# icdm-adteam/MoCoPCI

Hardware: AMD Instinct MI355X
Metric: interpolated frames/sec (higher is better)
Workload: dtype f32 (fused MLP layers: fp32 products as 6 bf16-MFMA partials of an exact 3-way split, fp32 accumulate; index paths exact f32)

## Files before the change

mocopci_amd/csrc/pointconv.hip:

```cpp
#include "common.h"
#include "mfma_split.h"

namespace {

constexpr int K = 32, WN = 8;

template <int THREADS, int PPB>
__global__ __launch_bounds__(THREADS) void pointconv_agg_kernel(long long total, int n, int s, int d, const float *__restrict__ s_xyz,
                                                                const float *__restrict__ new_xyz, const float *__restrict__ s_points,
                                                                const int *__restrict__ idx, const float *__restrict__ w0,
                                                                const float *__restrict__ b0, const float *__restrict__ w1,
                                                                const float *__restrict__ b1, const float *__restrict__ w2,
                                                                const float *__restrict__ b2, float *__restrict__ out) {
    __shared__ __attribute__((aligned(16))) float wl[PPB][K][WN];
    __shared__ float gx[PPB][K][3];
    __shared__ int il[PPB][K];
    const int tid = threadIdx.x;
    const int cin = d + 3;
    const bool f32 = mcp_fits32(total);
    const bool off32 = (long long)n * d < (1LL << 31);
    const int d4 = d >> 2;
    const McpUnits units = mcp_units_by_xcd(total, PPB);
    for (long long p0 = units.first; p0 < units.limit; p0 += units.stride) {
        __syncthreads();
        for (int pair = tid; pair < PPB * K; pair += THREADS) {
            const int pl = pair >> 5, k = pair & 31;
            const long long p = p0 + pl;
            if (p < total) {
                const long long bb = mcp_div(p, s, f32);
                const int id = idx[p * K + k];
                const float *q = s_xyz + ((long long)bb * n + id) * 3;
                const float x0 = q[0] - new_xyz[p * 3 + 0], x1 = q[1] - new_xyz[p * 3 + 1], x2 = q[2] - new_xyz[p * 3 + 2];
                float h0[WN], h1[WN], h2[WN];
#pragma unroll
                for (int j = 0; j < WN; ++j)
                    h0[j] = fmaxf(__builtin_fmaf(w0[j * 3 + 2], x2, __builtin_fmaf(w0[j * 3 + 1], x1, __builtin_fmaf(w0[j * 3], x0, b0[j]))), 0.f);
#pragma unroll
                for (int j = 0; j < WN; ++j) {
                    float a = b1[j];
#pragma unroll
                    for (int i = 0; i < WN; ++i) a = __builtin_fmaf(w1[j * WN + i], h0[i], a);
                    h1[j] = fmaxf(a, 0.f);
                }
#pragma unroll
                for (int j = 0; j < WN; ++j) {
                    float a = b2[j];
#pragma unroll
                    for (int i = 0; i < WN; ++i) a = __builtin_fmaf(w2[j * WN + i], h1[i], a);
                    h2[j] = fmaxf(a, 0.f);
                }
#pragma unroll
                for (int j = 0; j < WN; ++j) wl[pl][k][j] = h2[j];
                gx[pl][k][0] = x0; gx[pl][k][1] = x1; gx[pl][k][2] = x2;
                il[pl][k] = id;
            }
        }
        __syncthreads();
        for (int it = tid; it < PPB * d4; it += THREADS) {
            const int pl = it / d4, c = (it - pl * d4) * 4;
            const long long p = p0 + pl;
            if (p >= total) break;
            const long long bb = mcp_div(p, s, f32);
            float acc[4][WN];
#pragma unroll
            for (int u = 0; u < 4; ++u)
#pragma unroll
                for (int j = 0; j < WN; ++j) acc[u][j] = 0.f;
            const float *fb = s_points + (long long)bb * n * d + c;
#pragma unroll 8
            for (int k = 0; k < K; ++k) {
                const float4 f = *reinterpret_cast<const float4 *>(off32 ? fb + (unsigned)il[pl][k] * (unsigned)d : fb + (long long)il[pl][k] * d);
                const float4 wa = *reinterpret_cast<const float4 *>(&wl[pl][k][0]);
                const float4 wb = *reinterpret_cast<const float4 *>(&wl[pl][k][4]);
                const float fv[4] = {f.x, f.y, f.z, f.w};
#pragma unroll
                for (int u = 0; u < 4; ++u) {
                    acc[u][0] = __builtin_fmaf(fv[u], wa.x, acc[u][0]); acc[u][1] = __builtin_fmaf(fv[u], wa.y, acc[u][1]);
                    acc[u][2] = __builtin_fmaf(fv[u], wa.z, acc[u][2]); acc[u][3] = __builtin_fmaf(fv[u], wa.w, acc[u][3]);
                    acc[u][4] = __builtin_fmaf(fv[u], wb.x, acc[u][4]); acc[u][5] = __builtin_fmaf(fv[u], wb.y, acc[u][5]);
                    acc[u][6] = __builtin_fmaf(fv[u], wb.z, acc[u][6]); acc[u][7] = __builtin_fmaf(fv[u], wb.w, acc[u][7]);
                }
            }
            float4 *o = reinterpret_cast<float4 *>(out + (p * cin + 3 + c) * WN);
#pragma unroll
            for (int u = 0; u < 4; ++u) {
                o[2 * u] = make_float4(acc[u][0], acc[u][1], acc[u][2], acc[u][3]);
                o[2 * u + 1] = make_float4(acc[u][4], acc[u][5], acc[u][6], acc[u][7]);
            }
        }
        if (tid < PPB * 3) {
            const int pl = tid / 3, c = tid - pl * 3;
            const long long p = p0 + pl;
            if (p < total) {
                float acc[WN];
#pragma unroll
                for (int j = 0; j < WN; ++j) acc[j] = 0.f;
#pragma unroll 8
                for (int k = 0; k < K; ++k) {
                    const float f = gx[pl][k][c];
                    const float4 wa = *reinterpret_cast<const float4 *>(&wl[pl][k][0]);
                    const float4 wb = *reinterpret_cast<const float4 *>(&wl[pl][k][4]);
                    acc[0] = __builtin_fmaf(f, wa.x, acc[0]); acc[1] = __builtin_fmaf(f, wa.y, acc[1]);
                    acc[2] = __builtin_fmaf(f, wa.z, acc[2]); acc[3] = __builtin_fmaf(f, wa.w, acc[3]);
                    acc[4] = __builtin_fmaf(f, wb.x, acc[4]); acc[5] = __builtin_fmaf(f, wb.y, acc[5]);
                    acc[6] = __builtin_fmaf(f, wb.z, acc[6]); acc[7] = __builtin_fmaf(f, wb.w, acc[7]);
                }
                float4 *o = reinterpret_cast<float4 *>(out + (p * cin + c) * WN);
                o[0] = make_float4(acc[0], acc[1], acc[2], acc[3]);
                o[1] = make_float4(acc[4], acc[5], acc[6], acc[7]);
            }
        }
    }
}

constexpr int LPPB = 8;
template <int THREADS>
__global__ __launch_bounds__(THREADS) void pointconv_agg_lowlevel_kernel(long long total, int n, int s, int d, const float *__restrict__ s_xyz,
                                                                const float *__restrict__ new_xyz, const float *__restrict__ s_points,
                                                                const int *__restrict__ idx, const float *__restrict__ w0,
                                                                const float *__restrict__ b0, const float *__restrict__ w1,
                                                                const float *__restrict__ b1, const float *__restrict__ w2,
                                                                const float *__restrict__ b2, float *__restrict__ out) {
    __shared__ __attribute__((aligned(16))) float wl[LPPB][K][WN];
    __shared__ float gx[LPPB][K][3];
    __shared__ int il[LPPB][K];
    const int tid = threadIdx.x;
    const int cin = d + 3;
    const bool f32 = mcp_fits32(total);
    const bool off32 = (long long)n * d < (1LL << 31);
    const McpUnits units = mcp_units_by_xcd(total, LPPB);
    for (long long p0 = units.first; p0 < units.limit; p0 += units.stride) {
        __syncthreads();
        {
            const int pl = tid >> 5, k = tid & 31;
            const long long p = p0 + pl;
            if (tid < LPPB * K && p < total) {
                const long long bb = mcp_div(p, s, f32);
                const int id = idx[p * K + k];
                const float *q = s_xyz + ((long long)bb * n + id) * 3;
                const float x0 = q[0] - new_xyz[p * 3 + 0], x1 = q[1] - new_xyz[p * 3 + 1], x2 = q[2] - new_xyz[p * 3 + 2];
                float h0[WN], h1[WN], h2[WN];
#pragma unroll
                for (int j = 0; j < WN; ++j)
                    h0[j] = fmaxf(__builtin_fmaf(w0[j * 3 + 2], x2, __builtin_fmaf(w0[j * 3 + 1], x1, __builtin_fmaf(w0[j * 3], x0, b0[j]))), 0.f);
#pragma unroll
                for (int j = 0; j < WN; ++j) {
                    float a = b1[j];
#pragma unroll
                    for (int i = 0; i < WN; ++i) a = __builtin_fmaf(w1[j * WN + i], h0[i], a);
                    h1[j] = fmaxf(a, 0.f);
                }
#pragma unroll
                for (int j = 0; j < WN; ++j) {
                    float a = b2[j];
#pragma unroll
                    for (int i = 0; i < WN; ++i) a = __builtin_fmaf(w2[j * WN + i], h1[i], a);
                    h2[j] = fmaxf(a, 0.f);
                }
#pragma unroll
                for (int j = 0; j < WN; ++j) wl[pl][k][j] = h2[j];
                gx[pl][k][0] = x0; gx[pl][k][1] = x1; gx[pl][k][2] = x2;
                il[pl][k] = id;
            }
        }
        __syncthreads();
        for (int it = tid; it < LPPB * d; it += THREADS) {
            const int pl = it / d, c = it - pl * d;
            const long long p = p0 + pl;
            if (p >= total) break;
            const long long bb = mcp_div(p, s, f32);
            float acc[WN];
#pragma unroll
            for (int j = 0; j < WN; ++j) acc[j] = 0.f;
            const float *fb = s_points + (long long)bb * n * d + c;
#pragma unroll 8
            for (int k = 0; k < K; ++k) {
                const float f = off32 ? fb[(unsigned)il[pl][k] * (unsigned)d] : fb[(long long)il[pl][k] * d];
                const float4 wa = *reinterpret_cast<const float4 *>(&wl[pl][k][0]);
                const float4 wb = *reinterpret_cast<const float4 *>(&wl[pl][k][4]);
                acc[0] = __builtin_fmaf(f, wa.x, acc[0]); acc[1] = __builtin_fmaf(f, wa.y, acc[1]);
                acc[2] = __builtin_fmaf(f, wa.z, acc[2]); acc[3] = __builtin_fmaf(f, wa.w, acc[3]);
                acc[4] = __builtin_fmaf(f, wb.x, acc[4]); acc[5] = __builtin_fmaf(f, wb.y, acc[5]);
                acc[6] = __builtin_fmaf(f, wb.z, acc[6]); acc[7] = __builtin_fmaf(f, wb.w, acc[7]);
            }
            float4 *o = reinterpret_cast<float4 *>(out + (p * cin + 3 + c) * WN);
            o[0] = make_float4(acc[0], acc[1], acc[2], acc[3]);
            o[1] = make_float4(acc[4], acc[5], acc[6], acc[7]);
        }
        if (tid < LPPB * 3) {
            const int pl = tid / 3, c = tid - pl * 3;
            const long long p = p0 + pl;
            if (p < total) {
                float acc[WN];
#pragma unroll
                for (int j = 0; j < WN; ++j) acc[j] = 0.f;
#pragma unroll 8
                for (int k = 0; k < K; ++k) {
                    const float f = gx[pl][k][c];
                    const float4 wa = *reinterpret_cast<const float4 *>(&wl[pl][k][0]);
                    const float4 wb = *reinterpret_cast<const float4 *>(&wl[pl][k][4]);
                    acc[0] = __builtin_fmaf(f, wa.x, acc[0]); acc[1] = __builtin_fmaf(f, wa.y, acc[1]);
                    acc[2] = __builtin_fmaf(f, wa.z, acc[2]); acc[3] = __builtin_fmaf(f, wa.w, acc[3]);
                    acc[4] = __builtin_fmaf(f, wb.x, acc[4]); acc[5] = __builtin_fmaf(f, wb.y, acc[5]);
                    acc[6] = __builtin_fmaf(f, wb.z, acc[6]); acc[7] = __builtin_fmaf(f, wb.w, acc[7]);
                }
                float4 *o = reinterpret_cast<float4 *>(out + (p * cin + c) * WN);
                o[0] = make_float4(acc[0], acc[1], acc[2], acc[3]);
                o[1] = make_float4(acc[4], acc[5], acc[6], acc[7]);
            }
        }
    }
}

constexpr int FPPB = 32;
template <int D, int NT>
struct FusedCfg {
    static constexpr int THREADS = 8 * D;
    static constexpr int KTOT = 8 * D + 24, NCH = (KTOT + 31) / 32, KP = NCH * 32 + 4;
    static constexpr int SCRATCH_BYTES = FPPB * K * (WN + 3 + 1) * 4;
    static constexpr int TILE_BYTES = FPPB * KP * 4;
    static constexpr int XP = 36;
    static constexpr int STAGE_BYTES = NT * 32 * XP * 4;
    static constexpr int LDS_BYTES = (SCRATCH_BYTES > TILE_BYTES + STAGE_BYTES ? SCRATCH_BYTES : TILE_BYTES + STAGE_BYTES);
    static_assert(NT <= THREADS / 64, "one wave per output tile");
    static_assert(2 * LDS_BYTES <= 160 * 1024 || D < 64, "two workgroups per CU");
};

template <int D, int NT>
__global__ __launch_bounds__(8 * D) __attribute__((amdgpu_waves_per_eu(D == 32 ? 3 : 4))) void pointconv_linear_kernel(long long total, int n, int s, const float *__restrict__ s_xyz,
                                                                  const float *__restrict__ new_xyz, const float *__restrict__ s_points,
                                                                  const int *__restrict__ idx, const float *__restrict__ w0,
                                                                  const float *__restrict__ b0, const float *__restrict__ w1,
                                                                  const float *__restrict__ b1, const float *__restrict__ w2,
                                                                  const float *__restrict__ b2, const float *__restrict__ packed, int cout,
                                                                  float slope, float *__restrict__ out) {
    using C = FusedCfg<D, NT>;
    constexpr int THREADS = C::THREADS, NCH = C::NCH, KP = C::KP, KTOT = C::KTOT, D4 = D / 4, XP = C::XP;
    constexpr int CF = NT * 2 * 3 * 64 * 4;
    constexpr int UNR = D == 32 ? 4 : 2;
    extern __shared__ __attribute__((aligned(16))) float flds[];
    float(*wl)[K][WN] = reinterpret_cast<float(*)[K][WN]>(flds);
    float(*gx)[K][3] = reinterpret_cast<float(*)[K][3]>(flds + FPPB * K * WN);
    int(*il)[K] = reinterpret_cast<int(*)[K]>(flds + FPPB * K * (WN + 3));
    float *tile = flds;
    const int tid = threadIdx.x, lane = tid & 63, wave = tid >> 6, h = lane >> 5, col = lane & 31;
    const bool f32 = mcp_fits32(total);
    const bool off32 = (long long)n * D < (1LL << 31);
    const McpUnits units = mcp_units_by_xcd(total, FPPB);
    for (long long p0 = units.first; p0 < units.limit; p0 += units.stride) {
        __syncthreads();
        for (int pair = tid; pair < FPPB * K; pair += THREADS) {
            const int pl = pair >> 5, k = pair & 31;
            const long long p = p0 + pl;
            if (p < total) {
                const long long bb = mcp_div(p, s, f32);
                const int id = idx[p * K + k];
                const float *q = s_xyz + ((long long)bb * n + id) * 3;
                const float x0 = q[0] - new_xyz[p * 3 + 0], x1 = q[1] - new_xyz[p * 3 + 1], x2 = q[2] - new_xyz[p * 3 + 2];
                float h0[WN], h1[WN], h2[WN];
#pragma unroll
                for (int j = 0; j < WN; ++j)
                    h0[j] = fmaxf(__builtin_fmaf(w0[j * 3 + 2], x2, __builtin_fmaf(w0[j * 3 + 1], x1, __builtin_fmaf(w0[j * 3], x0, b0[j]))), 0.f);
#pragma unroll
                for (int j = 0; j < WN; ++j) {
                    float a = b1[j];
#pragma unroll
                    for (int i = 0; i < WN; ++i) a = __builtin_fmaf(w1[j * WN + i], h0[i], a);
                    h1[j] = fmaxf(a, 0.f);
                }
#pragma unroll
                for (int j = 0; j < WN; ++j) {
                    float a = b2[j];
#pragma unroll
                    for (int i = 0; i < WN; ++i) a = __builtin_fmaf(w2[j * WN + i], h1[i], a);
                    h2[j] = fmaxf(a, 0.f);
                }
#pragma unroll
                for (int j = 0; j < WN; ++j) wl[pl][k][j] = h2[j];
                gx[pl][k][0] = x0; gx[pl][k][1] = x1; gx[pl][k][2] = x2;
                il[pl][k] = id;
            }
        }
        __syncthreads();
        const int pl = tid / D4, c4 = tid - pl * D4;
        float acc[4][WN], accx[WN];
#pragma unroll
        for (int u = 0; u < 4; ++u)
#pragma unroll
            for (int j = 0; j < WN; ++j) acc[u][j] = 0.f;
#pragma unroll
        for (int j = 0; j < WN; ++j) accx[j] = 0.f;
        if (p0 + pl < total) {
            const long long bb = mcp_div(p0 + pl, s, f32);
            const float *fb = s_points + (long long)bb * n * D + c4 * 4;
#pragma unroll UNR
            for (int k = 0; k < K; ++k) {
                const float4 f = *reinterpret_cast<const float4 *>(off32 ? fb + (unsigned)il[pl][k] * (unsigned)D : fb + (long long)il[pl][k] * D);
                const float4 wa = *reinterpret_cast<const float4 *>(&wl[pl][k][0]);
                const float4 wb = *reinterpret_cast<const float4 *>(&wl[pl][k][4]);
                const float fv[4] = {f.x, f.y, f.z, f.w};
#pragma unroll
                for (int u = 0; u < 4; ++u) {
                    acc[u][0] = __builtin_fmaf(fv[u], wa.x, acc[u][0]); acc[u][1] = __builtin_fmaf(fv[u], wa.y, acc[u][1]);
                    acc[u][2] = __builtin_fmaf(fv[u], wa.z, acc[u][2]); acc[u][3] = __builtin_fmaf(fv[u], wa.w, acc[u][3]);
                    acc[u][4] = __builtin_fmaf(fv[u], wb.x, acc[u][4]); acc[u][5] = __builtin_fmaf(fv[u], wb.y, acc[u][5]);
                    acc[u][6] = __builtin_fmaf(fv[u], wb.z, acc[u][6]); acc[u][7] = __builtin_fmaf(fv[u], wb.w, acc[u][7]);
                }
            }
        }
        const int xl = tid / 3, xc = tid - xl * 3;
        if (tid < FPPB * 3 && p0 + xl < total) {
#pragma unroll UNR
            for (int k = 0; k < K; ++k) {
                const float f = gx[xl][k][xc];
                const float4 wa = *reinterpret_cast<const float4 *>(&wl[xl][k][0]);
                const float4 wb = *reinterpret_cast<const float4 *>(&wl[xl][k][4]);
                accx[0] = __builtin_fmaf(f, wa.x, accx[0]); accx[1] = __builtin_fmaf(f, wa.y, accx[1]);
                accx[2] = __builtin_fmaf(f, wa.z, accx[2]); accx[3] = __builtin_fmaf(f, wa.w, accx[3]);
                accx[4] = __builtin_fmaf(f, wb.x, accx[4]); accx[5] = __builtin_fmaf(f, wb.y, accx[5]);
                accx[6] = __builtin_fmaf(f, wb.z, accx[6]); accx[7] = __builtin_fmaf(f, wb.w, accx[7]);
            }
        }
        struct Wts { uint4 w[2][3]; };
        auto request = [&](int c, Wts &g) {
            const uint4 *wc = reinterpret_cast<const uint4 *>(packed + (size_t)min(c, NCH - 1) * CF) + (size_t)min(wave, NT - 1) * 2 * 3 * 64 + lane;
#pragma unroll
            for (int s2 = 0; s2 < 2; ++s2)
#pragma unroll
                for (int pc = 0; pc < 3; ++pc) g.w[s2][pc] = wc[(size_t)(s2 * 3 + pc) * 64];
        };
        Wts wa_;
        if (wave < NT) request(0, wa_);
        __syncthreads();
        {
            float *row = tile + pl * KP + 24 + c4 * 32;
#pragma unroll
            for (int u = 0; u < 4; ++u) {
                *reinterpret_cast<float4 *>(row + 8 * u) = make_float4(acc[u][0], acc[u][1], acc[u][2], acc[u][3]);
                *reinterpret_cast<float4 *>(row + 8 * u + 4) = make_float4(acc[u][4], acc[u][5], acc[u][6], acc[u][7]);
            }
            if (tid < FPPB * 3) {
                float *xr = tile + xl * KP + xc * 8;
                *reinterpret_cast<float4 *>(xr) = make_float4(accx[0], accx[1], accx[2], accx[3]);
                *reinterpret_cast<float4 *>(xr + 4) = make_float4(accx[4], accx[5], accx[6], accx[7]);
            } else if (tid < FPPB * 3 + FPPB) {
                float *xr = tile + (tid - FPPB * 3) * KP + KTOT;
#pragma unroll
                for (int i = 0; i < NCH * 32 - KTOT; i += 4) *reinterpret_cast<float4 *>(xr + i) = make_float4(0.f, 0.f, 0.f, 0.f);
            }
        }
        __syncthreads();
        if (wave < NT) {
            mcp_f32x16 o;
            {
                const float *bi = packed + (size_t)NCH * CF;
#pragma unroll
                for (int r = 0; r < 16; ++r) o[r] = bi[(wave * 2 + h) * 16 + r];
            }
#pragma unroll 1
            for (int c = 0; c < NCH; ++c) {
                mcp_f32x16 xa;
#pragma unroll
                for (int g = 0; g < 4; ++g) {
                    const float4 v = *reinterpret_cast<const float4 *>(tile + col * KP + c * 32 + 8 * g + 4 * h);
                    xa[4 * g + 0] = v.x; xa[4 * g + 1] = v.y; xa[4 * g + 2] = v.z; xa[4 * g + 3] = v.w;
                }
                McpSplit3 xs[2];
                xs[0] = mcp_split_kstep(xa, 0);
                xs[1] = mcp_split_kstep(xa, 1);
#pragma unroll
                for (int s2 = 0; s2 < 2; ++s2) {
                    o = mcp_mfma_bf16(wa_.w[s2][2], xs[s2].p1, o);
                    o = mcp_mfma_bf16(wa_.w[s2][0], xs[s2].p3, o);
                    o = mcp_mfma_bf16(wa_.w[s2][1], xs[s2].p2, o);
                    o = mcp_mfma_bf16(wa_.w[s2][1], xs[s2].p1, o);
                    o = mcp_mfma_bf16(wa_.w[s2][0], xs[s2].p2, o);
                    o = mcp_mfma_bf16(wa_.w[s2][0], xs[s2].p1, o);
                }
                request(c + 1, wa_);
            }
            float *st = flds + C::TILE_BYTES / 4 + wave * 32 * XP;
#pragma unroll
            for (int g = 0; g < 4; ++g) {
                float v[4];
#pragma unroll
                for (int u = 0; u < 4; ++u) {
                    const float a = o[4 * g + u];
                    v[u] = a > 0.f ? a : a * slope;
                }
                *reinterpret_cast<float4 *>(st + col * XP + 8 * g + 4 * h) = make_float4(v[0], v[1], v[2], v[3]);
            }
            const int cr = lane >> 3, cq = lane & 7;
#pragma unroll
            for (int j = 0; j < 4; ++j) {
                const long long p = p0 + 8 * j + cr;
                const float4 v4 = *reinterpret_cast<const float4 *>(st + (8 * j + cr) * XP + 4 * cq);
                if (p < total) *reinterpret_cast<float4 *>(out + p * cout + 32 * wave + 4 * cq) = v4;
            }
        }
    }
}

}

MCP_EXPORT int mcp_pointconv_agg(int b, int n, int s, int d, int k, const float *s_xyz, const float *new_xyz, const float *s_points,
                                 const int *idx, const float *w0, const float *b0, const float *w1, const float *b1, const float *w2,
                                 const float *b2, float *out, mcp_stream_t stream) {
    MCP_CHECK_ARGS(b > 0 && n > 0 && s > 0 && d > 0 && s_xyz && new_xyz && s_points && idx && w0 && b0 && w1 && b1 && w2 && b2 && out);
    if (k != K) return MCP_ERR_UNSUPPORTED;
    if (((uintptr_t)out) & 15) return MCP_ERR_BAD_ARG;
    hipStream_t st = (hipStream_t)stream;
    const long long total = (long long)b * s;
    const bool vec4 = !(d & 3) && !(((uintptr_t)s_points) & 15);
    mcp_prof_begin(MCP_KERNEL_POINTCONV, st);
    auto launch = [&](auto kern, int ppb) {
        const unsigned grid = (unsigned)min((total + ppb - 1) / ppb, 1LL << 20);
        hipLaunchKernelGGL(kern, dim3(grid), dim3(256), 0, st, total, n, s, d, s_xyz, new_xyz, s_points, idx, w0, b0, w1, b1, w2, b2, out);
    };
    if (total <= 16384 || !vec4) {
        const unsigned grid = (unsigned)min((total + LPPB - 1) / LPPB, 1LL << 20);
        if (d >= 256 && total <= 8192)
            hipLaunchKernelGGL(pointconv_agg_lowlevel_kernel<1024>, dim3(grid), dim3(1024), 0, st, total, n, s, d, s_xyz, new_xyz, s_points, idx, w0, b0, w1, b1, w2, b2, out);
        else
            hipLaunchKernelGGL(pointconv_agg_lowlevel_kernel<256>, dim3(grid), dim3(256), 0, st, total, n, s, d, s_xyz, new_xyz, s_points, idx, w0, b0, w1, b1, w2, b2, out);
    } else if (d <= 32) launch(pointconv_agg_kernel<256, 32>, 32);
    else if (d <= 64) launch(pointconv_agg_kernel<256, 16>, 16);
    else launch(pointconv_agg_kernel<256, 8>, 8);
    mcp_prof_end(MCP_KERNEL_POINTCONV, st);
    return mcp_launch_status();
}

MCP_EXPORT int mcp_pointconv_linear(int b, int n, int s, int d, int k, const float *s_xyz, const float *new_xyz, const float *s_points,
                                    const int *idx, const float *w0, const float *b0, const float *w1, const float *b1, const float *w2,
                                    const float *b2, const float *packed, int c_out, float slope, float *out, mcp_stream_t stream) {
    MCP_CHECK_ARGS(b > 0 && n > 0 && s > 0 && d > 0 && s_xyz && new_xyz && s_points && idx && w0 && b0 && w1 && b1 && w2 && b2 && packed && out);
    if (k != K || !((d == 32 && c_out == 32) || (d == 64 && c_out == 64))) return MCP_ERR_UNSUPPORTED;
    if ((((uintptr_t)out) | ((uintptr_t)s_points) | ((uintptr_t)packed)) & 15) return MCP_ERR_BAD_ARG;
    hipStream_t st = (hipStream_t)stream;
    const long long total = (long long)b * s;
    const unsigned grid = (unsigned)min((total + FPPB - 1) / FPPB, 1LL << 20);
    mcp_prof_begin(MCP_KERNEL_POINTCONV, st);
    if (d == 32) {
        auto kern = pointconv_linear_kernel<32, 1>;
        static McpPerDeviceOnce attr_once;
        if (attr_once.need()) {
            { const hipError_t attr_e_ = hipFuncSetAttribute(reinterpret_cast<const void *>(kern), hipFuncAttributeMaxDynamicSharedMemorySize, 160 * 1024); if (attr_e_ != hipSuccess) return (int)attr_e_; }
            attr_once.done();
        }
        constexpr int lds = FusedCfg<32, 1>::LDS_BYTES;
        hipLaunchKernelGGL(kern, dim3(grid), dim3(256), lds, st, total, n, s, s_xyz, new_xyz, s_points, idx, w0, b0, w1, b1, w2,
                           b2, packed, c_out, slope, out);
    } else {
        auto kern = pointconv_linear_kernel<64, 2>;
        static McpPerDeviceOnce attr_once;
        if (attr_once.need()) {
            { const hipError_t attr_e_ = hipFuncSetAttribute(reinterpret_cast<const void *>(kern), hipFuncAttributeMaxDynamicSharedMemorySize, 160 * 1024); if (attr_e_ != hipSuccess) return (int)attr_e_; }
            attr_once.done();
        }
        constexpr int lds = FusedCfg<64, 2>::LDS_BYTES;
        hipLaunchKernelGGL(kern, dim3(grid), dim3(512), lds, st, total, n, s, s_xyz, new_xyz, s_points, idx, w0, b0, w1, b1, w2,
                           b2, packed, c_out, slope, out);
    }
    mcp_prof_end(MCP_KERNEL_POINTCONV, st);
    return mcp_launch_status();
}
```

Measured before the change: 3539.

## Software-pipeline neighbor feature gathers and split coordinate accumulation across threads

Replaces the per-neighbor gather loop with a register ring that prefetches G groups of four float4 neighbor rows ahead of their FMAs, using sched_barrier fences and int4 index loads so global-load latency overlaps with compute. The MLP prologue now issues all idx, centre and neighbor-xyz loads up front before computing. The xyz-weighted accumulation is split over six threads per point, each doing half the weights, to shorten that serial phase. The ring raises register pressure, and the off32 fallback for large offsets is dropped in favour of size_t arithmetic.

```diff
diff --git a/mocopci_amd/csrc/pointconv.hip b/mocopci_amd/csrc/pointconv.hip
--- a/mocopci_amd/csrc/pointconv.hip
+++ b/mocopci_amd/csrc/pointconv.hip
@@ -226,6 +226,56 @@
     static_assert(2 * LDS_BYTES <= 160 * 1024 || D < 64, "two workgroups per CU");
 };
 
+__device__ __forceinline__ int mcp_pc_opaque(int v) {
+    asm volatile("" : "+v"(v));
+    return v;
+}
+
+template <int D, int G>
+__device__ __forceinline__ void pointconv_agg_ring(const float *__restrict__ fb, const int *ilp, const float *wlp, float (&acc)[4][WN]) {
+    constexpr int NG = K / 4;
+    constexpr int RING_FENCE = 0x184;
+    static_assert(NG % G == 0 && G < NG, "the ring turns a whole number of times");
+    const int4 *ilq = reinterpret_cast<const int4 *>(ilp);
+    auto gather = [&](int id) { return *reinterpret_cast<const float4 *>(fb + (size_t)(unsigned)id * D); };
+    auto fma_row = [&](const float4 &f, int k) {
+        const float4 wa = *reinterpret_cast<const float4 *>(wlp + k * WN);
+        const float4 wb = *reinterpret_cast<const float4 *>(wlp + k * WN + 4);
+        const float fv[4] = {f.x, f.y, f.z, f.w};
+#pragma unroll
+        for (int u = 0; u < 4; ++u) {
+            acc[u][0] = __builtin_fmaf(fv[u], wa.x, acc[u][0]); acc[u][1] = __builtin_fmaf(fv[u], wa.y, acc[u][1]);
+            acc[u][2] = __builtin_fmaf(fv[u], wa.z, acc[u][2]); acc[u][3] = __builtin_fmaf(fv[u], wa.w, acc[u][3]);
+            acc[u][4] = __builtin_fmaf(fv[u], wb.x, acc[u][4]); acc[u][5] = __builtin_fmaf(fv[u], wb.y, acc[u][5]);
+            acc[u][6] = __builtin_fmaf(fv[u], wb.z, acc[u][6]); acc[u][7] = __builtin_fmaf(fv[u], wb.w, acc[u][7]);
+        }
+    };
+    float4 r[G][4];
+#pragma unroll
+    for (int g = 0; g < G; ++g) {
+        const int4 id = ilq[g];
+        r[g][0] = gather(id.x); r[g][1] = gather(id.y); r[g][2] = gather(id.z); r[g][3] = gather(id.w);
+    }
+    int4 nx = ilq[G];
+#pragma unroll 1
+    for (int g0 = 0; g0 < NG - G; g0 += G) {
+#pragma unroll
+        for (int gg = 0; gg < G; ++gg) {
+            const int g = g0 + gg;
+            const int4 id = nx;
+            nx = ilq[min(g + G + 1, NG - 1)];
+            fma_row(r[gg][0], 4 * g + 0); r[gg][0] = gather(id.x); __builtin_amdgcn_sched_barrier(RING_FENCE);
+            fma_row(r[gg][1], 4 * g + 1); r[gg][1] = gather(id.y); __builtin_amdgcn_sched_barrier(RING_FENCE);
+            fma_row(r[gg][2], 4 * g + 2); r[gg][2] = gather(id.z); __builtin_amdgcn_sched_barrier(RING_FENCE);
+            fma_row(r[gg][3], 4 * g + 3); r[gg][3] = gather(id.w); __builtin_amdgcn_sched_barrier(RING_FENCE);
+        }
+    }
+#pragma unroll
+    for (int gg = 0; gg < G; ++gg)
+#pragma unroll
+        for (int j = 0; j < 4; ++j) fma_row(r[gg][j], 4 * (NG - G + gg) + j);
+}
+
 template <int D, int NT>
 __global__ __launch_bounds__(8 * D) __attribute__((amdgpu_waves_per_eu(D == 32 ? 3 : 4))) void pointconv_linear_kernel(long long total, int n, int s, const float *__restrict__ s_xyz,
                                                                   const float *__restrict__ new_xyz, const float *__restrict__ s_points,
@@ -237,26 +287,42 @@
     using C = FusedCfg<D, NT>;
     constexpr int THREADS = C::THREADS, NCH = C::NCH, KP = C::KP, KTOT = C::KTOT, D4 = D / 4, XP = C::XP;
     constexpr int CF = NT * 2 * 3 * 64 * 4;
-    constexpr int UNR = D == 32 ? 4 : 2;
+    constexpr int RING = D == 32 ? 4 : 1;
+    constexpr int XUNR = 8;
+    static_assert(FPPB * 6 + FPPB <= THREADS, "coordinate channels and the padding on distinct threads");
     extern __shared__ __attribute__((aligned(16))) float flds[];
     float(*wl)[K][WN] = reinterpret_cast<float(*)[K][WN]>(flds);
     float(*gx)[K][3] = reinterpret_cast<float(*)[K][3]>(flds + FPPB * K * WN);
     int(*il)[K] = reinterpret_cast<int(*)[K]>(flds + FPPB * K * (WN + 3));
     float *tile = flds;
-    const int tid = threadIdx.x, lane = tid & 63, wave = tid >> 6, h = lane >> 5, col = lane & 31;
+    const int tid = threadIdx.x;
     const bool f32 = mcp_fits32(total);
-    const bool off32 = (long long)n * D < (1LL << 31);
     const McpUnits units = mcp_units_by_xcd(total, FPPB);
     for (long long p0 = units.first; p0 < units.limit; p0 += units.stride) {
         __syncthreads();
-        for (int pair = tid; pair < FPPB * K; pair += THREADS) {
-            const int pl = pair >> 5, k = pair & 31;
-            const long long p = p0 + pl;
-            if (p < total) {
-                const long long bb = mcp_div(p, s, f32);
-                const int id = idx[p * K + k];
-                const float *q = s_xyz + ((long long)bb * n + id) * 3;
-                const float x0 = q[0] - new_xyz[p * 3 + 0], x1 = q[1] - new_xyz[p * 3 + 1], x2 = q[2] - new_xyz[p * 3 + 2];
+        constexpr int NP = FPPB * K / THREADS, PSTEP = THREADS / K;
+        const int t1 = mcp_pc_opaque(tid), pl1 = t1 >> 5, k = t1 & 31;
+        int ids[NP];
+        float cx[NP][3], qx[NP][3];
+#pragma unroll
+        for (int i = 0; i < NP; ++i) {
+            const long long p = min(p0 + pl1 + i * PSTEP, total - 1);
+            ids[i] = idx[p * K + k];
+#pragma unroll
+            for (int a = 0; a < 3; ++a) cx[i][a] = new_xyz[p * 3 + a];
+        }
+#pragma unroll
+        for (int i = 0; i < NP; ++i) {
+            const long long p = min(p0 + pl1 + i * PSTEP, total - 1);
+            const float *q = s_xyz + (mcp_div(p, s, f32) * n + ids[i]) * 3;
+#pragma unroll
+            for (int a = 0; a < 3; ++a) qx[i][a] = q[a];
+        }
+#pragma unroll
+        for (int e = 0; e < NP; ++e) {
+            const int pl = pl1 + e * PSTEP, id = ids[e];
+            if (p0 + pl < total) {
+                const float x0 = qx[e][0] - cx[e][0], x1 = qx[e][1] - cx[e][1], x2 = qx[e][2] - cx[e][2];
                 float h0[WN], h1[WN], h2[WN];
 #pragma unroll
                 for (int j = 0; j < WN; ++j)
@@ -282,45 +348,29 @@
             }
         }
         __syncthreads();
-        const int pl = tid / D4, c4 = tid - pl * D4;
-        float acc[4][WN], accx[WN];
+        const int t2 = mcp_pc_opaque(tid);
+        const int pl = t2 / D4, c4 = t2 - pl * D4;
+        float acc[4][WN], accx[4] = {0.f, 0.f, 0.f, 0.f};
 #pragma unroll
         for (int u = 0; u < 4; ++u)
 #pragma unroll
             for (int j = 0; j < WN; ++j) acc[u][j] = 0.f;
-#pragma unroll
-        for (int j = 0; j < WN; ++j) accx[j] = 0.f;
         if (p0 + pl < total) {
             const long long bb = mcp_div(p0 + pl, s, f32);
             const float *fb = s_points + (long long)bb * n * D + c4 * 4;
-#pragma unroll UNR
-            for (int k = 0; k < K; ++k) {
-                const float4 f = *reinterpret_cast<const float4 *>(off32 ? fb + (unsigned)il[pl][k] * (unsigned)D : fb + (long long)il[pl][k] * D);
-                const float4 wa = *reinterpret_cast<const float4 *>(&wl[pl][k][0]);
-                const float4 wb = *reinterpret_cast<const float4 *>(&wl[pl][k][4]);
-                const float fv[4] = {f.x, f.y, f.z, f.w};
-#pragma unroll
-                for (int u = 0; u < 4; ++u) {
-                    acc[u][0] = __builtin_fmaf(fv[u], wa.x, acc[u][0]); acc[u][1] = __builtin_fmaf(fv[u], wa.y, acc[u][1]);
-                    acc[u][2] = __builtin_fmaf(fv[u], wa.z, acc[u][2]); acc[u][3] = __builtin_fmaf(fv[u], wa.w, acc[u][3]);
-                    acc[u][4] = __builtin_fmaf(fv[u], wb.x, acc[u][4]); acc[u][5] = __builtin_fmaf(fv[u], wb.y, acc[u][5]);
-                    acc[u][6] = __builtin_fmaf(fv[u], wb.z, acc[u][6]); acc[u][7] = __builtin_fmaf(fv[u], wb.w, acc[u][7]);
-                }
-            }
-        }
-        const int xl = tid / 3, xc = tid - xl * 3;
-        if (tid < FPPB * 3 && p0 + xl < total) {
-#pragma unroll UNR
+            pointconv_agg_ring<D, RING>(fb, &il[pl][0], &wl[pl][0][0], acc);
+        }
+        const int xl = t2 / 6, xq = t2 - xl * 6, xc = xq >> 1, xh = xq & 1;
+        if (t2 < FPPB * 6 && p0 + xl < total) {
+#pragma unroll XUNR
             for (int k = 0; k < K; ++k) {
                 const float f = gx[xl][k][xc];
-                const float4 wa = *reinterpret_cast<const float4 *>(&wl[xl][k][0]);
-                const float4 wb = *reinterpret_cast<const float4 *>(&wl[xl][k][4]);
-                accx[0] = __builtin_fmaf(f, wa.x, accx[0]); accx[1] = __builtin_fmaf(f, wa.y, accx[1]);
-                accx[2] = __builtin_fmaf(f, wa.z, accx[2]); accx[3] = __builtin_fmaf(f, wa.w, accx[3]);
-                accx[4] = __builtin_fmaf(f, wb.x, accx[4]); accx[5] = __builtin_fmaf(f, wb.y, accx[5]);
-                accx[6] = __builtin_fmaf(f, wb.z, accx[6]); accx[7] = __builtin_fmaf(f, wb.w, accx[7]);
-            }
-        }
+                const float4 w = *reinterpret_cast<const float4 *>(&wl[xl][k][4 * xh]);
+                accx[0] = __builtin_fmaf(f, w.x, accx[0]); accx[1] = __builtin_fmaf(f, w.y, accx[1]);
+                accx[2] = __builtin_fmaf(f, w.z, accx[2]); accx[3] = __builtin_fmaf(f, w.w, accx[3]);
+            }
+        }
+        const int t3 = mcp_pc_opaque(tid), lane = t3 & 63, wave = t3 >> 6, h = lane >> 5, col = lane & 31;
         struct Wts { uint4 w[2][3]; };
         auto request = [&](int c, Wts &g) {
             const uint4 *wc = reinterpret_cast<const uint4 *>(packed + (size_t)min(c, NCH - 1) * CF) + (size_t)min(wave, NT - 1) * 2 * 3 * 64 + lane;
@@ -339,12 +389,10 @@
                 *reinterpret_cast<float4 *>(row + 8 * u) = make_float4(acc[u][0], acc[u][1], acc[u][2], acc[u][3]);
                 *reinterpret_cast<float4 *>(row + 8 * u + 4) = make_float4(acc[u][4], acc[u][5], acc[u][6], acc[u][7]);
             }
-            if (tid < FPPB * 3) {
-                float *xr = tile + xl * KP + xc * 8;
-                *reinterpret_cast<float4 *>(xr) = make_float4(accx[0], accx[1], accx[2], accx[3]);
-                *reinterpret_cast<float4 *>(xr + 4) = make_float4(accx[4], accx[5], accx[6], accx[7]);
-            } else if (tid < FPPB * 3 + FPPB) {
-                float *xr = tile + (tid - FPPB * 3) * KP + KTOT;
+            if (t2 < FPPB * 6) {
+                *reinterpret_cast<float4 *>(tile + xl * KP + xc * 8 + xh * 4) = make_float4(accx[0], accx[1], accx[2], accx[3]);
+            } else if (t2 < FPPB * 6 + FPPB) {
+                float *xr = tile + (t2 - FPPB * 6) * KP + KTOT;
 #pragma unroll
                 for (int i = 0; i < NCH * 32 - KTOT; i += 4) *reinterpret_cast<float4 *>(xr + i) = make_float4(0.f, 0.f, 0.f, 0.f);
             }
```

After: 3520. No clear change (-0.5%).
